# UCSC-nanopore-cgl/margin

Hardware: AMD Instinct MI355X
Metric: het-sites x reads phased/sec (30x ONT synthetic chunks, end to end: every merge level + final sweep) (higher is better)
Workload: dtype int32

## Files before the change

margin_amd/csrc/mrp_batch.cpp:

```cpp
#include <hip/hip_runtime.h>

#include <algorithm>
#include <array>
#include <cstdio>
#include <cstdlib>
#include <cstring>
#include <ctime>
#include <mutex>
#include <new>
#include <vector>

#include "mrp_internal.h"
#include "mrp_level_order.h"

extern "C" {

int mrp_batch_create(mrp_context *ctx, mrp_batch **out) {
    if (!ctx || !out) return mrp_set_error(MRP_ERR_ARG, "mrp_batch_create: bad arguments");
    mrp_batch *b = new (std::nothrow) mrp_batch();
    if (!b) return mrp_set_error(MRP_ERR_NOMEM, "out of host memory");
    b->ctx = ctx;
    b->bind_pool(&ctx->pool);
    *out = b;
    return MRP_OK;
// ... 332 lines not shown
    for (size_t i = 0; i < b->pcols.size(); i++) (b->pcols[i].need_planes ? plane_list : pack_list).push_back((int32_t) i);
    HIP_TRY(b->d_pack_list.upload(pack_list, s));
    HIP_TRY(b->d_plane_list.upload(plane_list, s));
    const double u3 = now_();
    const size_t nC = (size_t) b->n_cells_total;
    HIP_TRY(b->d_planes.alloc((size_t) b->n_slots * 8));
    HIP_TRY(b->d_slot_total.alloc((size_t) b->n_slots));
    HIP_TRY(b->d_slot_bytes.alloc((size_t) b->n_slots * 16));
    HIP_TRY(b->d_cost.alloc(nC));
    HIP_TRY(b->d_f32.alloc(nC));
    HIP_TRY(b->d_b32.alloc(nC));
    HIP_TRY(b->d_mf32.alloc((size_t) b->n_merge));
    HIP_TRY(b->d_mb32.alloc((size_t) b->n_merge));
    if (!b->order_f64.empty()) {
        HIP_TRY(b->d_f.alloc(nC));
        HIP_TRY(b->d_b.alloc(nC));
        HIP_TRY(b->d_mf.alloc((size_t) b->n_merge));
        HIP_TRY(b->d_mb.alloc((size_t) b->n_merge));
    }
    HIP_TRY(b->d_total.alloc(b->cols.size()));
    HIP_TRY(b->d_hmm_fb.alloc(2 * b->hmms.size()));
    const double u4 = now_();
    HIP_TRY(hipStreamSynchronize(s));
    if (timing_)
        fprintf(stderr, "      upload: plan %.2f ms, arrays %.2f, tiles+lists %.2f, allocs %.2f, sync %.2f\n", u1 - u0, u2 - u1, u3 - u2, u4 - u3, now_() - u4);

    b->dev = b->view();
    HostVec<int64_t>().swap(b->read_byte_off);
    HostVec<uint64_t>().swap(b->partition);
    HostVec<uint32_t>().swap(b->cell_next);
    HostVec<uint32_t>().swap(b->cell_prev);
    HostVec<uint32_t>().swap(b->cell_np);
    b->uploaded = true;
    return MRP_OK;
}

int mrp_batch_launch(mrp_batch *b) {
    if (!b) return mrp_set_error(MRP_ERR_ARG, "batch is NULL");
    if (!b->uploaded) {
        int rc = mrp_batch_upload(b);
        if (rc != MRP_OK) return rc;
    }
    mrp_context *ctx = b->ctx;
    HIP_TRY(hipSetDevice(ctx->device));
    hipStream_t s = ctx->stream;
    const MrpBatchDev &d = b->dev;
    hipStream_t ps = s;
    const size_t slot = (size_t) (b->n_launches % mrp_batch::EV_RING);
    if (slot >= b->ev_ring.size()) {
        std::array<hipEvent_t, 5> fresh{};
        for (auto &ev : fresh) HIP_TRY(hipEventCreate(&ev));
        b->ev_ring.push_back(fresh);
    }
    const std::array<hipEvent_t, 5> &ev = b->ev_ring[slot];
    if (b->n_launches >= mrp_batch::EV_RING) HIP_TRY(hipEventSynchronize(ev[2]));
    if (ps != s && ctx->last_emission) HIP_TRY(hipStreamWaitEvent(ps, ctx->last_emission, 0));
    HIP_TRY(hipEventRecord(ev[0], ps));
    HIP_TRY(mrp_launch_planes(d, ps));
    if (b->resident && mrp_dup('p')) HIP_TRY(mrp_launch_planes(d, ps));
    HIP_TRY(hipEventRecord(ev[1], ps));
    if (ps != s) HIP_TRY(hipStreamWaitEvent(s, ev[1], 0));
    HIP_TRY(hipEventRecord(ev[4], s));
    if (b->pre_sweep) HIP_TRY(b->pre_sweep(s));
    if (b->pre_sweep && mrp_dup('x')) HIP_TRY(b->pre_sweep(s));
    HIP_TRY(mrp_launch_emission(d, b->d_tiles.p, b->n_fast_tiles, b->n_tiles_dev - b->n_fast_tiles, s));
    HIP_TRY(hipEventRecord(ev[3], s));
    ctx->last_emission = ev[3];
    if (!b->order_f64.empty()) {
        const double neg = -__builtin_inf();
        HIP_TRY(mrp_launch_fill_f64(b->d_mf.p, d.n_merge, neg, s));
        HIP_TRY(mrp_launch_fill_f64(b->d_mb.p, d.n_merge, neg, s));
        HIP_TRY(mrp_launch_fill_f64(b->d_total.p, d.n_cols, neg, s));
        HIP_TRY(mrp_launch_fill_f64(b->d_hmm_fb.p, 2 * d.n_hmms, neg, s));
    }
    hipStream_t a0 = s, a1 = s;
    if (s == ctx->stream) HIP_TRY(ctx->side_streams(&a0, &a1));
    const bool side = a0 != s;
    if (side) {
        HIP_TRY(hipEventRecord(ctx->fork, s));
        HIP_TRY(hipStreamWaitEvent(a0, ctx->fork, 0));
        HIP_TRY(hipStreamWaitEvent(a1, ctx->fork, 0));
    }
    const int64_t chains = 2 * (int64_t) (b->order_wide.size() + b->order_mid.size()) * (int64_t) ctx->concurrent_batches;
    const int t_chain = ctx->concurrent_batches > 1 && chains > 2 * 256 ? 256 : 512;
    const int t_wide = t_chain, t_mid = t_chain, t_narrow = 64;
    HIP_TRY(mrp_launch_sweep_i32(d, b->d_order_wide.p, (int64_t) b->order_wide.size(), t_wide, b->max_merge_wide, s));
    HIP_TRY(mrp_launch_sweep_i32(d, b->d_order_mid.p, (int64_t) b->order_mid.size(), t_mid, b->max_merge_mid, a0));
    HIP_TRY(mrp_launch_sweep_i32(d, b->d_order_narrow.p, (int64_t) b->order_narrow.size(), t_narrow, b->max_merge_narrow, a1));
    if (b->resident && mrp_dup('s')) {
        HIP_TRY(mrp_launch_sweep_i32(d, b->d_order_wide.p, (int64_t) b->order_wide.size(), t_wide, b->max_merge_wide, s));
        HIP_TRY(mrp_launch_sweep_i32(d, b->d_order_mid.p, (int64_t) b->order_mid.size(), t_mid, b->max_merge_mid, a0));
        HIP_TRY(mrp_launch_sweep_i32(d, b->d_order_narrow.p, (int64_t) b->order_narrow.size(), t_narrow, b->max_merge_narrow, a1));
    }
    HIP_TRY(mrp_launch_sweep_f64(d, b->d_order_f64.p, (int64_t) b->order_gen.size(), 256, s));
    HIP_TRY(mrp_launch_sweep_lse(d, b->d_order_lse.p, (int64_t) b->order_lse.size(), b->max_merge_lse, s));
    HIP_TRY(mrp_launch_sweep_lse(d, b->d_order_lse_big.p, (int64_t) b->order_lse_big.size(), std::max(b->max_merge_lse_big, MRP_LSE_CUR_LDS_MAX_MERGE + 2), s));
    if (side) {
        HIP_TRY(hipEventRecord(ctx->join[0], a0));
        HIP_TRY(hipEventRecord(ctx->join[1], a1));
        HIP_TRY(hipStreamWaitEvent(s, ctx->join[0], 0));
        HIP_TRY(hipStreamWaitEvent(s, ctx->join[1], 0));
    }
    HIP_TRY(hipEventRecord(ev[2], s));
    b->n_launches++;
    b->launched = true;
    return MRP_OK;
}

int mrp_batch_stats(mrp_batch *b, mrp_launch_stats *out) {
    if (!b || !out) return mrp_set_error(MRP_ERR_ARG, "mrp_batch_stats: NULL argument");
    *out = b->stats;
    out->n_hmms_lse = (int64_t) (b->order_lse.size() + b->order_lse_big.size());
    out->n_hmms_generic = (int64_t) b->order_gen.size();
    out->n_hmms_int32 = (int64_t) (b->order_wide.size() + b->order_mid.size() + b->order_narrow.size());
    if (b->launched) {
        mrp_context *ctx = b->ctx;
        HIP_TRY(hipSetDevice(ctx->device));
        const int64_t k = std::min<int64_t>(std::max<int64_t>(b->n_launches - b->stats_mark, 1), std::min<int64_t>(b->n_launches, mrp_batch::EV_RING));
        b->stats_mark = b->n_launches;
        double sa = 0, se = 0, sc = 0;
        float a = 0, e = 0, c = 0;
        for (int64_t j = 0; j < k; j++) {
            const auto &ev = b->ev_ring[(size_t) ((b->n_launches - k + j) % mrp_batch::EV_RING)];
            HIP_TRY(hipEventSynchronize(ev[2]));
            HIP_TRY(hipEventElapsedTime(&a, ev[0], ev[1]));
            HIP_TRY(hipEventElapsedTime(&e, ev[4], ev[3]));
            HIP_TRY(hipEventElapsedTime(&c, ev[3], ev[2]));
            sa += a; se += e; sc += c;
        }
        out->planes_ms = a;
        out->emission_ms = e;
        out->sweep_ms = c;
        out->avg_planes_ms = k ? sa / (double) k : 0.0;
        out->avg_emission_ms = k ? se / (double) k : 0.0;
        out->avg_sweep_ms = k ? sc / (double) k : 0.0;
        out->launches_averaged = k;
    }
    return MRP_OK;
}

void mrp_batch_last_launch_ms(mrp_batch *b, float *pack, float *emission, float *recursion) {
    *pack = *emission = *recursion = 0.f;
    if (!b || !b->launched || b->n_launches < 1) return;
    const auto &ev = b->ev_ring[(size_t) ((b->n_launches - 1) % mrp_batch::EV_RING)];
    (void) hipEventElapsedTime(pack, ev[0], ev[1]);
    (void) hipEventElapsedTime(emission, ev[4], ev[3]);
    (void) hipEventElapsedTime(recursion, ev[3], ev[2]);
}

int mrp_batch_download(mrp_batch *b) {
    if (!b) return mrp_set_error(MRP_ERR_ARG, "batch is NULL");
    if (!b->launched) return mrp_set_error(MRP_ERR_ARG, "mrp_batch_download before mrp_batch_launch");
    mrp_context *ctx = b->ctx;
    HIP_TRY(hipSetDevice(ctx->device));
    hipStream_t s = ctx->stream;
    const MrpBatchDev &d = b->dev;
    const bool any_out = std::any_of(b->outs.begin(), b->outs.end(), [](const JobOut &o) { return o.cell_f != nullptr; });
    if (!any_out) {
        HIP_TRY(hipStreamSynchronize(s));
        return MRP_OK;
    }
    const bool has_f64 = !b->order_f64.empty();
    std::vector<double> f, bb, mf, mb, tot((size_t) d.n_cols), fb((size_t) (2 * d.n_hmms));
    std::vector<int32_t> f32((size_t) d.n_cells), b32((size_t) d.n_cells), mf32((size_t) d.n_merge), mb32((size_t) d.n_merge);
    if (has_f64) { f.resize((size_t) d.n_cells); bb.resize((size_t) d.n_cells); mf.resize((size_t) d.n_merge); mb.resize((size_t) d.n_merge); }
    auto pull = [&](void *h, const void *p, size_t bytes) -> hipError_t {
        if (bytes == 0) return hipSuccess;
// ... 159 lines not shown
```

margin_amd/csrc/mrp_context.cpp:

```cpp
#include <hip/hip_runtime.h>

#include <atomic>
#include <cstdarg>
#include <cstdio>
#include <cstdlib>
#include <mutex>
#include <new>

#include "mrp_internal.h"

static thread_local char g_err[512] = "";

extern "C" {

int mrp_set_error(int code, const char *fmt, ...) {
    va_list ap;
    va_start(ap, fmt);
    vsnprintf(g_err, sizeof(g_err), fmt, ap);
    va_end(ap);
    return code;
}

const char *mrp_last_error(void) { return g_err; }
const char *mrp_version(void) { return "margin_rphmm 0.5.0 gfx950"; }
// ... 41 lines not shown
    *device_held = ctx->pool.device >= 0 ? (int64_t) DevPoolRegistry::get().held[ctx->pool.device].load() : 0;
}
mrp_context *mrp_context_sibling(mrp_context *ctx, int i) {
    std::lock_guard<std::mutex> lock(ctx->sibling_mu);
    while ((int) ctx->siblings.size() <= i) {
        mrp_context *s = nullptr;
        if (mrp_context_create(ctx->device, &s) != MRP_OK) return nullptr;
        s->phase_groups = 1;
        s->grouped = true;
        s->test_hooks = ctx->test_hooks;
        ctx->siblings.push_back(s);
    }
    return ctx->siblings[(size_t) i];
}
int mrp_context_create(int device, mrp_context **out) {
    if (!out) return mrp_set_error(MRP_ERR_ARG, "mrp_context_create: out is NULL");
    *out = nullptr;
    int n = mrp_device_count();
    if (n <= 0) return mrp_set_error(MRP_ERR_NO_DEVICE, "no HIP device visible: the stRPHmm sweep has no CPU fallback");
    if (device < 0 || device >= n) return mrp_set_error(MRP_ERR_ARG, "device %d out of range (0..%d)", device, n - 1);
    HIP_TRY(hipSetDevice(device));
    mrp_context *ctx = new (std::nothrow) mrp_context();
    if (!ctx) return mrp_set_error(MRP_ERR_NOMEM, "out of host memory");
    ctx->device = device;
    ctx->pool.attach(device);
    hipError_t e = hipStreamCreateWithFlags(&ctx->stream, hipStreamNonBlocking);
    for (int i = 0; i < 4 && e == hipSuccess; i++) e = hipEventCreate(&ctx->ev[i]);
    if (e == hipSuccess) e = hipEventCreateWithFlags(&ctx->fork, hipEventDisableTiming);
    for (int i = 0; i < 2 && e == hipSuccess; i++) e = hipEventCreateWithFlags(&ctx->join[i], hipEventDisableTiming);
    if (e != hipSuccess) {
        mrp_context_destroy(ctx);
        return mrp_set_error(MRP_ERR_HIP, "context setup failed: %s", hipGetErrorString(e));
    }
    *out = ctx;
    return MRP_OK;
}

void mrp_context_destroy(mrp_context *ctx) {
    if (!ctx) return;
    for (mrp_context *s : ctx->siblings) mrp_context_destroy(s);
    ctx->siblings.clear();
    (void) hipSetDevice(ctx->device);
    mrp_engine_release_context_cache(ctx);
    (void) hipDeviceSynchronize();
    ctx->pool.destroy();
    for (auto &e : ctx->ev)
        if (e) (void) hipEventDestroy(e);
    if (ctx->fork) (void) hipEventDestroy(ctx->fork);
    if (ctx->block_ev) (void) hipEventDestroy(ctx->block_ev);
    for (auto &e : ctx->join)
        if (e) (void) hipEventDestroy(e);
    for (auto &st : ctx->aux)
        if (st) (void) hipStreamDestroy(st);
    if (ctx->pre) (void) hipStreamDestroy(ctx->pre);
    if (ctx->stream) (void) hipStreamDestroy(ctx->stream);
    delete ctx;
}

int mrp_context_trim(mrp_context *ctx) {
    if (!ctx) return mrp_set_error(MRP_ERR_ARG, "context is NULL");
    HIP_TRY(hipSetDevice(ctx->device));
    HIP_TRY(hipDeviceSynchronize());
    std::lock_guard<std::mutex> lock(ctx->sibling_mu);
    for (mrp_context *s_ : ctx->siblings) { s_->pool.reclaim(); s_->pool.trim(); }
    ctx->pool.reclaim();
    ctx->pool.trim();
    DevPoolRegistry::get().forget_budget(ctx->pool.device);
    return MRP_OK;
}

int mrp_context_synchronize(mrp_context *ctx) {
    if (!ctx) return mrp_set_error(MRP_ERR_ARG, "context is NULL");
    HIP_TRY(hipSetDevice(ctx->device));
    HIP_TRY(hipStreamSynchronize(ctx->stream));
    return MRP_OK;
}
int mrp_context_set_phase_groups(mrp_context *ctx, int groups) {
    if (!ctx || groups < 0 || groups > 16) return mrp_set_error(MRP_ERR_ARG, "mrp_context_set_phase_groups: bad arguments");
    ctx->phase_groups = groups;
    return MRP_OK;
}
int mrp_context_phase_groups(const mrp_context *ctx) { return ctx->phase_groups; }
int mrp_context_set_test_hooks(mrp_context *ctx, int hooks) {
    if (!ctx || hooks < 0 || hooks > 63) return mrp_set_error(MRP_ERR_ARG, "mrp_context_set_test_hooks: bad arguments");
    if ((hooks & 4) && ctx->pool.device >= 0) DevPoolRegistry::get().inject_oom[ctx->pool.device].store(1);
    hooks &= ~4;
    ctx->test_hooks = hooks;
    for (mrp_context *s_ : ctx->siblings) s_->test_hooks = hooks;
    return MRP_OK;
}
int mrp_context_test_hooks(const mrp_context *ctx) { return ctx->test_hooks; }

}
```

margin_amd/csrc/mrp_kernels.hip:

```cpp
#include <hip/hip_runtime.h>
#include <stdint.h>

#include "mrp_device.h"
#include "mrp_internal.h"
#include "mrp_kernels.h"
#include "../../include/margin_rphmm.h"

#define WAVE 64

#define K_AS(T) const __attribute__((address_space(4))) T *
#define K_PTR(T, p) ((K_AS(T)) (p))
template <typename T>
static __device__ __forceinline__ T k_load(const T *p) {
    static_assert(sizeof(T) % 4 == 0, "dword sized");
    T v;
    K_AS(uint32_t) s = K_PTR(uint32_t, p);
    uint32_t *dst = reinterpret_cast<uint32_t *>(&v);
#pragma unroll
    for (unsigned i = 0; i < sizeof(T) / 4; i++) dst[i] = s[i];
    return v;
}

static __device__ __forceinline__ double i32_to_log(int32_t v) {
    return v == MRP_NEG_I32 ? -__builtin_inf() : (double) v;
// ... 314 lines not shown
__global__ void __launch_bounds__(256) mrp_emission_kernel(MrpBatchDev d, const EmitTile *__restrict__ tiles,
                                                           int64_t n_tiles) {
    const int lane = threadIdx.x & (WAVE - 1);
    const int wave = __builtin_amdgcn_readfirstlane((int) (threadIdx.x / WAVE));
    const int64_t tile = (int64_t) blockIdx.x * (blockDim.x / WAVE) + wave;
    if (tile >= n_tiles) return;
    const EmitTile t = k_load(tiles + tile);
    if (t.depth <= 16) emit_tile<4, 4>(d, t, lane, 0);
    else if (t.depth <= 32) emit_tile<8, 4>(d, t, lane, 0);
    else if (t.depth <= 48) {
        emit_tile<12, 2>(d, t, lane, 0);
        if (t.n > 256) emit_tile<12, 2>(d, t, lane, 128);
    } else {
        emit_tile<16, 2>(d, t, lane, 0);
        if (t.n > 256) emit_tile<16, 2>(d, t, lane, 128);
    }
}

__global__ void __launch_bounds__(256) mrp_emission_general_kernel(MrpBatchDev d, const EmitTile *__restrict__ tiles,
                                                                   int64_t n_tiles) {
    const int lane = threadIdx.x & (WAVE - 1);
    const int wave = __builtin_amdgcn_readfirstlane((int) (threadIdx.x / WAVE));
    const int64_t tile = (int64_t) blockIdx.x * (blockDim.x / WAVE) + wave;
    if (tile >= n_tiles) return;
    const EmitTile t = k_load(tiles + tile);
    const DevCol c = k_load(d.cols + t.col);
    const DevChunk ch = k_load(d.chunks + c.chunk);
    K_AS(uint64_t) planes = K_PTR(uint64_t, d.planes);
    K_AS(uint32_t) slot_total = K_PTR(uint32_t, d.slot_total);
    const bool ancestor = (t.flags & MRP_FLAG_INCLUDE_ANCESTOR_SUB_PROB) != 0;
    for (int idx = lane; idx < t.n; idx += WAVE) {
        const uint64_t P[1] = {d.partition[t.cell_off + idx]};
        uint32_t cost[1];
        if (ancestor) cost[0] = column_cost_ancestor(c, ch, planes, slot_total, P[0]);
        else column_cost_plain<1, false>(c, K_PTR(uint32_t, ch.allele_number), planes, slot_total, P, cost);
        d.cell_cost[t.cell_off + idx] = cost[0];
    }
}

__global__ void __launch_bounds__(256) mrp_tiles_kernel(const DevCol *__restrict__ cols, const TileCol *__restrict__ tc, int64_t n_cols,
                                                        EmitTile *__restrict__ tiles) {
    const int64_t col = (int64_t) blockIdx.x * blockDim.x + threadIdx.x;
    if (col >= n_cols) return;
    const DevCol c = cols[col];
    const TileCol t0 = tc[col];
    int64_t at = t0.first;
    for (int32_t off = 0; off < c.n_cells; off += MRP_EMIT_TILE, at++) {
        EmitTile t;
        t.cell_off = c.cell_off + off;
        t.slot_off = c.slot_off;
        t.n = c.n_cells - off < MRP_EMIT_TILE ? c.n_cells - off : MRP_EMIT_TILE;
        t.col = (int32_t) col;
        t.n_sites = c.n_sites;
        t.uniform_alleles = t0.uniform_alleles;
        t.depth = c.depth;
        t.flags = c.flags;
        t.pad[0] = 0;
        t.pad[1] = 0;
        tiles[at] = t;
    }
}

hipError_t mrp_launch_tiles(const DevCol *cols_dev, const TileCol *tilecols_dev, int64_t n_cols, EmitTile *tiles_dev, hipStream_t stream) {
    if (n_cols <= 0) return hipSuccess;
    hipLaunchKernelGGL(mrp_tiles_kernel, dim3((unsigned) ((n_cols + 255) / 256)), dim3(256), 0, stream, cols_dev, tilecols_dev, n_cols, tiles_dev);
    return hipGetLastError();
}

hipError_t mrp_launch_emission(const MrpBatchDev &d, const EmitTile *tiles_dev, int64_t n_fast, int64_t n_general,
                               hipStream_t stream) {
    const int waves = 4;
    if (n_fast > 0)
        hipLaunchKernelGGL(mrp_emission_kernel, dim3((unsigned) ((n_fast + waves - 1) / waves)), dim3(waves * WAVE), 0,
                           stream, d, tiles_dev, n_fast);
    if (n_general > 0)
        hipLaunchKernelGGL(mrp_emission_general_kernel, dim3((unsigned) ((n_general + waves - 1) / waves)),
                           dim3(waves * WAVE), 0, stream, d, tiles_dev + n_fast, n_general);
    return hipGetLastError();
}

#define SWEEP_R 8
#define SWEEP_WIN 128

struct SweepShared {
    int32_t *cur;
    int32_t *nxt;
    int32_t *red;
    int2 *dsc;
    int win0;
};

static __device__ __forceinline__ void stage_window(SweepShared &S, const SweepCol *cols, int K, int win0, int tid, int T) {
    __syncthreads();
    for (int i = tid; i < SWEEP_WIN; i += T) {
        const int k = win0 + i;
        if (k >= 0 && k < K) S.dsc[i] = make_int2(cols[k].n_cells, cols[k].n_merge);
    }
    S.win0 = win0;
    __syncthreads();
}
static __device__ __forceinline__ int2 col_desc(const SweepShared &S, int k) {
    const int2 v = S.dsc[k - S.win0];
    return make_int2(__builtin_amdgcn_readfirstlane(v.x), __builtin_amdgcn_readfirstlane(v.y));
}

__global__ void __launch_bounds__(1024)
mrp_sweep_i32_kernel(MrpBatchDev d, const int32_t *__restrict__ order, int max_merge) {
    extern __shared__ __attribute__((aligned(16))) int32_t lds[];
    SweepShared S;
    S.cur = lds;
    S.nxt = lds + max_merge;
    S.red = lds + 2 * max_merge;
    S.dsc = reinterpret_cast<int2 *>(lds + 2 * max_merge + 4);
    S.win0 = 0;

    const int tid = threadIdx.x, T = blockDim.x, lane = threadIdx.x & (WAVE - 1);
    const bool backward = (blockIdx.x & 1) != 0;
    const int64_t hmm_index = K_PTR(int32_t, order)[blockIdx.x >> 1];
    const DevHmm h = k_load(d.hmms + hmm_index);
    const SweepCol *cols = d.scols + h.col0;
    const int K = h.n_cols;
    const SweepCol first_col = k_load(cols);
    const int N = (int) h.n_cells;
    const int G = (N + 3) / 4;
    const int Q = (G + T - 1) / T;
    const uint32_t *__restrict__ cost = d.cell_cost + first_col.cell_off;
    const uint32_t *__restrict__ np = d.cell_np + first_col.cell_off;
    int32_t *__restrict__ out_f = d.cell_f32 + first_col.cell_off;
    int32_t *__restrict__ out_b = d.cell_b32 + first_col.cell_off;
    int32_t *__restrict__ out_mf = d.merge_f32 + first_col.mcell_off;
    int32_t *__restrict__ out_mb = d.merge_b32 + first_col.mcell_off;

    typedef uint32_t u32x4 __attribute__((ext_vector_type(4)));
    typedef int32_t i32x4 __attribute__((ext_vector_type(4)));
    u32x4 rc0, rc1, rc2, rc3, rc4, rc5, rc6, rc7, rn0, rn1, rn2, rn3, rn4, rn5, rn6, rn7;
#define RING_LOAD(i, q)                                                                              \
    {                                                                                                \
        int g_ = (q) * T + tid;                                                                      \
        g_ = g_ < 0 ? 0 : (g_ > G - 1 ? G - 1 : g_);                                                 \
        asm volatile("global_load_dwordx4 %0, %2, off\n\tglobal_load_dwordx4 %1, %3, off"            \
                     : "=&v"(rc##i), "=&v"(rn##i)                                                    \
                     : "v"(cost + 4 * g_), "v"(np + 4 * g_)                                          \
                     : "memory");                                                                    \
    }
#ifdef MRP_SAFE_WAIT
#define RING_WAIT(i, n) asm volatile("s_waitcnt vmcnt(0)" : "+v"(rc##i), "+v"(rn##i)::"memory");
#else
#define RING_WAIT(i, n) asm volatile("s_waitcnt vmcnt(" #n ")" : "+v"(rc##i), "+v"(rn##i)::"memory");
#endif
    if (!backward) {
        RING_LOAD(0, 0) RING_LOAD(1, 1) RING_LOAD(2, 2) RING_LOAD(3, 3)
        RING_LOAD(4, 4) RING_LOAD(5, 5) RING_LOAD(6, 6) RING_LOAD(7, 7)
    } else {
        RING_LOAD(0, Q - 1) RING_LOAD(1, Q - 2) RING_LOAD(2, Q - 3) RING_LOAD(3, Q - 4)
        RING_LOAD(4, Q - 5) RING_LOAD(5, Q - 6) RING_LOAD(6, Q - 7) RING_LOAD(7, Q - 8)
    }

    for (int i = tid; i < 2 * max_merge; i += T) lds[i] = MRP_NEG_I32;
    if (tid < 4) S.red[tid] = MRP_NEG_I32;
    stage_window(S, cols, K, 0, tid, T);

#define STORE4(out, p0, ok, v)                                                                               \
    {                                                                                                        \
        int32_t *dst_ = (ok) ? (out) + (p0) : scratch;                                                       \
        const i32x4 q_ = {v[0], v[1], v[2], v[3]};                                                           \
        *reinterpret_cast<i32x4 *>(dst_) = q_;                                                               \
    }
    int32_t *scratch = d.cell_f32 + d.n_cells;

#define RING_DRAIN() asm volatile("s_waitcnt vmcnt(0)"                                                                          \
                 : "+v"(rc0), "+v"(rc1), "+v"(rc2), "+v"(rc3), "+v"(rc4), "+v"(rc5), "+v"(rc6), "+v"(rc7),       \
                   "+v"(rn0), "+v"(rn1), "+v"(rn2), "+v"(rn3), "+v"(rn4), "+v"(rn5), "+v"(rn6), "+v"(rn7)        \
                 :                                                                                             \
                 : "memory");

    if (!backward) {
        int k = 0;
        int2 dk = col_desc(S, 0);
        int cs = 0, ce = dk.x;
        int mo = 0;
        int32_t local_max = MRP_NEG_I32;
#define FWD_ROUND(i, qq, nw)                                                                               \
    RING_WAIT(i, nw)                                                                                         \
    {                                                                                                        \
    const int pos0 = 4 * ((qq) * T + tid);                                                                   \
    int32_t fv[4] = {MRP_NEG_I32, MRP_NEG_I32, MRP_NEG_I32, MRP_NEG_I32};                                    \
    if ((qq) < Q && k < K) {                                                                                 \
        const int rend = 4 * ((qq) + 1) * T;                                                                 \
        for (;;) {                                                                                           \
            const bool first = (k == 0), last = (k == K - 1);                                                \
                        \
            bool act[4];                                                                                     \
            bool any_act = false;                                                                            \
            _Pragma("unroll") for (int j = 0; j < 4; j++) {                                                  \
                const int p = pos0 + j;                                                                      \
                act[j] = (p >= cs) & (p < ce);                                                               \
                any_act |= act[j];                                                                           \
            }                                                                                                \
            if (__any(any_act)) {                                                                            \
                int32_t fp[4] = {0, 0, 0, 0};                                                                \
                if (!first) {                                                                                \
                    _Pragma("unroll") for (int j = 0; j < 4; j++)                                            \
                        fp[j] = S.cur[act[j] ? (rn##i[j] >> 16) : lane];           \
                }                                                                                            \
                _Pragma("unroll") for (int j = 0; j < 4; j++) {                                              \
                    const int32_t v = add_i32(fp[j], -(int32_t) rc##i[j]);                                   \
                    fv[j] = act[j] ? v : fv[j];                                                              \
                    const int32_t val = act[j] ? v : MRP_NEG_I32;                                            \
                    if (!last) atomicMax(&S.nxt[act[j] ? (rn##i[j] & 0xFFFFu) : lane], val);       \
                    else local_max = max(local_max, val);                                                    \
                }                                                                                            \
            }                                                                                                \
            if (ce > rend) break;                                \
                                                                                   \
            if (last) {                                                                                      \
                local_max = wave_max_i32(local_max);                                                         \
                if ((tid & (WAVE - 1)) == 0) atomicMax(&S.red[0], local_max);                                \
                k = K;                                                                                       \
                break;                                                                                       \
            }                                                                                                \
            if (k + 1 >= S.win0 + SWEEP_WIN) stage_window(S, cols, K, k, tid, T);                            \
            const int2 dn = col_desc(S, k + 1);                                                              \
            lds_barrier();                                                                                   \
            for (int m = tid; m < dk.y; m += T) out_mf[mo + m] = S.nxt[m];                       \
            if (k + 2 < K) for (int m = tid; m < dn.y; m += T) S.cur[m] = MRP_NEG_I32;                       \
            lds_barrier();                                                                                   \
            { int32_t *t_ = S.cur; S.cur = S.nxt; S.nxt = t_; }                                              \
            mo += dk.y;                                                                                      \
            k++;                                                                                             \
            dk = dn;                                                                                         \
            cs = ce;                                                                                         \
            ce = cs + dk.x;                                                                                  \
            if (cs >= rend) break;                                                                           \
        }                                                                                                    \
    }                                                                                                        \
    STORE4(out_f, pos0, (qq) < Q && pos0 < N, fv)                                                            \
    }                                                                                                        \
    RING_LOAD(i, (qq) + SWEEP_R)
        FWD_ROUND(0, 0, 14) FWD_ROUND(1, 1, 15) FWD_ROUND(2, 2, 16) FWD_ROUND(3, 3, 17)
        FWD_ROUND(4, 4, 18) FWD_ROUND(5, 5, 19) FWD_ROUND(6, 6, 20) FWD_ROUND(7, 7, 21)
        for (int q0 = SWEEP_R; q0 < Q; q0 += SWEEP_R) {
            FWD_ROUND(0, q0, 21) FWD_ROUND(1, q0 + 1, 21) FWD_ROUND(2, q0 + 2, 21) FWD_ROUND(3, q0 + 3, 21)
            FWD_ROUND(4, q0 + 4, 21) FWD_ROUND(5, q0 + 5, 21) FWD_ROUND(6, q0 + 6, 21) FWD_ROUND(7, q0 + 7, 21)
        }
#undef FWD_ROUND
        RING_DRAIN()
        __syncthreads();
        const double total = i32_to_log(S.red[0]);
        for (int kk = tid; kk < K; kk += T) d.col_total[h.col0 + kk] = total;
        if (tid == 0) d.hmm_fb[2 * hmm_index] = total;
    }
    else {
        int k = K - 1;
        if (k < S.win0 || k >= S.win0 + SWEEP_WIN) stage_window(S, cols, K, max(0, K - SWEEP_WIN), tid, T);
        int2 dk = col_desc(S, k);
        int ce = N, cs = N - dk.x;
        int mo = (int) h.n_merge;
        if (K >= 2) {
            if (k - 1 < S.win0) stage_window(S, cols, K, max(0, k - SWEEP_WIN + 1), tid, T);
            const int2 dp = col_desc(S, k - 1);
            for (int m = tid; m < dp.y; m += T) S.nxt[m] = MRP_NEG_I32;
        }
        lds_barrier();
        int32_t local_max = MRP_NEG_I32;
#define BWD_ROUND(i, qq, nw)                                                                                 \
    RING_WAIT(i, nw)                                                                                         \
    {                                                                                                        \
    const int pos0 = 4 * ((qq) * T + tid);                                                                   \
    int32_t bv[4] = {MRP_NEG_I32, MRP_NEG_I32, MRP_NEG_I32, MRP_NEG_I32};                                    \
    if ((qq) >= 0 && k >= 0) {                                                                               \
        const int rbeg = 4 * (qq) * T;                                                                       \
        for (;;) {                                                                                           \
            const bool first = (k == 0), last = (k == K - 1);                                                \
            bool act[4];                                                                                     \
            bool any_act = false;                                                                            \
            _Pragma("unroll") for (int j = 0; j < 4; j++) {                                                  \
                const int p = pos0 + j;                                                                      \
                act[j] = (p >= cs) & (p < ce);                                                               \
                any_act |= act[j];                                                                           \
            }                                                                                                \
            if (__any(any_act)) {                                                                            \
                int32_t bn[4] = {0, 0, 0, 0};                                                                \
                if (!last) {                                                                                 \
                    _Pragma("unroll") for (int j = 0; j < 4; j++)                                            \
                        bn[j] = S.cur[act[j] ? (rn##i[j] & 0xFFFFu) : lane];       \
                }                                                                                            \
                _Pragma("unroll") for (int j = 0; j < 4; j++) {                                              \
                    bv[j] = act[j] ? bn[j] : bv[j];                                                          \
                    const int32_t pv = act[j] ? add_i32(bn[j], -(int32_t) rc##i[j]) : MRP_NEG_I32;           \
                    if (!first) atomicMax(&S.nxt[act[j] ? (rn##i[j] >> 16) : lane], pv);                     \
                    else local_max = max(local_max, pv);                                                     \
                }                                                                                            \
            }                                                                                                \
            if (cs < rbeg) break;                            \
            if (first) {                                                                                     \
                local_max = wave_max_i32(local_max);                                                         \
                if ((tid & (WAVE - 1)) == 0) atomicMax(&S.red[1], local_max);                                \
                k = -1;                                                                                      \
                break;                                                                                       \
            }                                                                                                \
            if (k - 2 >= 0 && k - 2 < S.win0) stage_window(S, cols, K, max(0, k - SWEEP_WIN + 1), tid, T);   \
            else if (k - 1 < S.win0) stage_window(S, cols, K, max(0, k - SWEEP_WIN + 1), tid, T);            \
            const int2 dp = col_desc(S, k - 1);                                                              \
            const int n_clear = (k >= 2) ? col_desc(S, k - 2).y : 0;                                         \
            lds_barrier();                                                                                   \
            for (int m = tid; m < dp.y; m += T) out_mb[mo - dp.y + m] = S.nxt[m];                \
            for (int m = tid; m < n_clear; m += T) S.cur[m] = MRP_NEG_I32;                                   \
            lds_barrier();                                                                                   \
            { int32_t *t_ = S.cur; S.cur = S.nxt; S.nxt = t_; }                                              \
            mo -= dp.y;                                                                                      \
            k--;                                                                                             \
            dk = dp;                                                                                         \
            ce = cs;                                                                                         \
            cs = ce - dk.x;                                                                                  \
            if (ce <= rbeg) break;                                                                           \
        }                                                                                                    \
    }                                                                                                        \
    STORE4(out_b, pos0, (qq) >= 0 && pos0 < N, bv)                                                           \
    }                                                                                                        \
    RING_LOAD(i, (qq) - SWEEP_R)
        BWD_ROUND(0, Q - 1, 14) BWD_ROUND(1, Q - 2, 15) BWD_ROUND(2, Q - 3, 16) BWD_ROUND(3, Q - 4, 17)
        BWD_ROUND(4, Q - 5, 18) BWD_ROUND(5, Q - 6, 19) BWD_ROUND(6, Q - 7, 20) BWD_ROUND(7, Q - 8, 21)
        for (int q0 = Q - 1 - SWEEP_R; q0 >= 0; q0 -= SWEEP_R) {
            BWD_ROUND(0, q0, 21) BWD_ROUND(1, q0 - 1, 21) BWD_ROUND(2, q0 - 2, 21) BWD_ROUND(3, q0 - 3, 21)
            BWD_ROUND(4, q0 - 4, 21) BWD_ROUND(5, q0 - 5, 21) BWD_ROUND(6, q0 - 6, 21) BWD_ROUND(7, q0 - 7, 21)
        }
#undef BWD_ROUND
        RING_DRAIN()
        __syncthreads();
        if (tid == 0) d.hmm_fb[2 * hmm_index + 1] = i32_to_log(S.red[1]);
    }
#undef RING_DRAIN
#undef RING_LOAD
#undef RING_WAIT
#undef STORE4
}

hipError_t mrp_launch_sweep_i32(const MrpBatchDev &d, const int32_t *order_dev, int64_t n, int block_threads,
                                int max_merge, hipStream_t stream) {
    if (n == 0) return hipSuccess;
    if (max_merge < WAVE) max_merge = WAVE;
    const size_t lds = (size_t) (2 * max_merge + 4) * sizeof(int32_t) + SWEEP_WIN * sizeof(int2);
    auto k = mrp_sweep_i32_kernel;
    static PerDeviceOnce once;
    const hipError_t attr_status = once.run([] {
        return hipFuncSetAttribute((const void *) mrp_sweep_i32_kernel, hipFuncAttributeMaxDynamicSharedMemorySize, 160 * 1024);
    });
    if (attr_status != hipSuccess) return attr_status;
    hipLaunchKernelGGL(k, dim3((unsigned) (2 * n)), dim3(block_threads), lds, stream, d, order_dev, max_merge);
    return hipGetLastError();
}

static __device__ __forceinline__ double log_add_exact(double x, double y) {
    if (x == -__builtin_inf()) return y;
    if (y == -__builtin_inf()) return x;
    return x > y ? x + log(1.0 + exp(y - x)) : y + log(1.0 + exp(x - y));
}
static __device__ __forceinline__ double log_add_p(double a, double b, bool max_not_sum) {
    return max_not_sum ? (a > b ? a : b) : log_add_exact(a, b);
}
static __device__ __forceinline__ double load_agent(double *p) {
    return __hip_atomic_load(p, __ATOMIC_RELAXED, __HIP_MEMORY_SCOPE_AGENT);
}
static __device__ void atomic_log_add_p(double *addr, double v, bool max_not_sum) {
    if (v == -__builtin_inf()) return;
    unsigned long long *a = (unsigned long long *) addr;
    unsigned long long old = __hip_atomic_load(a, __ATOMIC_RELAXED, __HIP_MEMORY_SCOPE_AGENT);
    while (true) {
        const double cur = __longlong_as_double((long long) old);
        const double nv = log_add_p(cur, v, max_not_sum);
        const unsigned long long nvb = (unsigned long long) __double_as_longlong(nv);
        if (nvb == old) return;
        const unsigned long long seen = atomicCAS(a, old, nvb);
        if (seen == old) return;
        old = seen;
    }
}
static __device__ __forceinline__ double wave_log_add_p(double v, bool max_not_sum) {
#pragma unroll
    for (int o = 32; o > 0; o >>= 1) {
        const double t = __shfl_xor(v, o, WAVE);
        v = log_add_p(v, t, max_not_sum);
    }
    return v;
}

__global__ void __launch_bounds__(1024) mrp_sweep_f64_kernel(MrpBatchDev d, const int32_t *__restrict__ order) {
    const int tid = threadIdx.x, T = blockDim.x;
    const int64_t hmm_index = K_PTR(int32_t, order)[blockIdx.x];
    const DevHmm h = k_load(d.hmms + hmm_index);
    const SweepCol *cols = d.scols + h.col0;
    const int K = h.n_cols;
    const bool wide = h.wide_idx != 0;
    const bool max_not_sum = (h.flags & MRP_FLAG_MAX_NOT_SUM) != 0;
    const double NEG = -__builtin_inf();
    double *hmm_f = d.hmm_fb + 2 * hmm_index, *hmm_b = hmm_f + 1;

    for (int k = 0; k < K; k++) {
        const SweepCol c = k_load(cols + k);
        const bool first = (k == 0), last = (k == K - 1);
        const SweepCol pc = k_load(cols + (first ? k : k - 1));
        double local = NEG;
        for (int idx = tid; idx < c.n_cells; idx += T) {
            const int64_t g = c.cell_off + idx;
            const double e = -((double) d.cell_cost[g]);
            const uint32_t nx = wide ? d.cell_next[g] : (d.cell_np[g] & 0xFFFFu);
            const uint32_t pv = wide ? d.cell_prev[g] : (d.cell_np[g] >> 16);
            double fv = first ? 0.0 : load_agent(&d.merge_f[pc.mcell_off + pv]);
            fv += e;
            d.cell_f[g] = fv;
            if (!last) atomic_log_add_p(&d.merge_f[c.mcell_off + nx], fv, max_not_sum);
            else local = log_add_p(local, fv, max_not_sum);
        }
        if (last) {
            local = wave_log_add_p(local, max_not_sum);
            if ((tid & (WAVE - 1)) == 0) atomic_log_add_p(hmm_f, local, max_not_sum);
        }
        __syncthreads();
    }
    for (int k = K - 1; k >= 0; k--) {
        const SweepCol c = k_load(cols + k);
        const bool first = (k == 0), last = (k == K - 1);
        const SweepCol pc = k_load(cols + (first ? k : k - 1));
        double local_b = NEG, local_t = NEG;
        for (int idx = tid; idx < c.n_cells; idx += T) {
            const int64_t g = c.cell_off + idx;
            const uint32_t nx = wide ? d.cell_next[g] : (d.cell_np[g] & 0xFFFFu);
            const uint32_t pv = wide ? d.cell_prev[g] : (d.cell_np[g] >> 16);
            double p = -((double) d.cell_cost[g]);
            double bv = 0.0;
            if (!last) { bv = load_agent(&d.merge_b[c.mcell_off + nx]); p += bv; }
            d.cell_b[g] = bv;
            if (!first) atomic_log_add_p(&d.merge_b[pc.mcell_off + pv], p, max_not_sum);
// ... 198 lines not shown
```

Before: 416.5 million.

## Template i32 sweep kernel on block size and direction, keep column descriptors in registers

The i32 forward/backward sweep kernel is templated on block size and direction, with separate launch instantiations for 64, 256 and 512 threads. Column descriptors now sit in a per-wave register window filled by inline-asm global loads and read via readlane, with a three-column lookahead. This replaces the LDS staging window and the block-wide barriers it needed, and the per-cell work is split into edge and non-edge template variants so interior columns skip the first/last checks. It also adds a test hook that forces 256-thread chains, and it raises register pressure and adds a synchronous load wait inside the loop.

Result: faster. 437.5 million, median of 5 (+5.0%).

```diff
diff --git a/margin_amd/csrc/mrp_batch.cpp b/margin_amd/csrc/mrp_batch.cpp
--- a/margin_amd/csrc/mrp_batch.cpp
+++ b/margin_amd/csrc/mrp_batch.cpp
@@ -438,7 +438,7 @@
         HIP_TRY(hipStreamWaitEvent(a1, ctx->fork, 0));
     }
     const int64_t chains = 2 * (int64_t) (b->order_wide.size() + b->order_mid.size()) * (int64_t) ctx->concurrent_batches;
-    const int t_chain = ctx->concurrent_batches > 1 && chains > 2 * 256 ? 256 : 512;
+    const int t_chain = (ctx->test_hooks & 64) || (ctx->concurrent_batches > 1 && chains > 2 * 256) ? 256 : 512;
     const int t_wide = t_chain, t_mid = t_chain, t_narrow = 64;
     HIP_TRY(mrp_launch_sweep_i32(d, b->d_order_wide.p, (int64_t) b->order_wide.size(), t_wide, b->max_merge_wide, s));
     HIP_TRY(mrp_launch_sweep_i32(d, b->d_order_mid.p, (int64_t) b->order_mid.size(), t_mid, b->max_merge_mid, a0));
diff --git a/margin_amd/csrc/mrp_context.cpp b/margin_amd/csrc/mrp_context.cpp
--- a/margin_amd/csrc/mrp_context.cpp
+++ b/margin_amd/csrc/mrp_context.cpp
@@ -147,7 +147,7 @@
 }
 int mrp_context_phase_groups(const mrp_context *ctx) { return ctx->phase_groups; }
 int mrp_context_set_test_hooks(mrp_context *ctx, int hooks) {
-    if (!ctx || hooks < 0 || hooks > 63) return mrp_set_error(MRP_ERR_ARG, "mrp_context_set_test_hooks: bad arguments");
+    if (!ctx || hooks < 0 || hooks > 127) return mrp_set_error(MRP_ERR_ARG, "mrp_context_set_test_hooks: bad arguments");
     if ((hooks & 4) && ctx->pool.device >= 0) DevPoolRegistry::get().inject_oom[ctx->pool.device].store(1);
     hooks &= ~4;
     ctx->test_hooks = hooks;
diff --git a/margin_amd/csrc/mrp_kernels.hip b/margin_amd/csrc/mrp_kernels.hip
--- a/margin_amd/csrc/mrp_kernels.hip
+++ b/margin_amd/csrc/mrp_kernels.hip
@@ -420,40 +420,84 @@
 #define SWEEP_R 8
 #define SWEEP_WIN 128
 
-struct SweepShared {
-    int32_t *cur;
-    int32_t *nxt;
-    int32_t *red;
-    int2 *dsc;
-    int win0;
-};
-
-static __device__ __forceinline__ void stage_window(SweepShared &S, const SweepCol *cols, int K, int win0, int tid, int T) {
-    __syncthreads();
-    for (int i = tid; i < SWEEP_WIN; i += T) {
-        const int k = win0 + i;
-        if (k >= 0 && k < K) S.dsc[i] = make_int2(cols[k].n_cells, cols[k].n_merge);
-    }
-    S.win0 = win0;
-    __syncthreads();
-}
-static __device__ __forceinline__ int2 col_desc(const SweepShared &S, int k) {
-    const int2 v = S.dsc[k - S.win0];
-    return make_int2(__builtin_amdgcn_readfirstlane(v.x), __builtin_amdgcn_readfirstlane(v.y));
-}
-
-__global__ void __launch_bounds__(1024)
-mrp_sweep_i32_kernel(MrpBatchDev d, const int32_t *__restrict__ order, int max_merge) {
+typedef uint32_t u32x4 __attribute__((ext_vector_type(4)));
+typedef int32_t i32x4 __attribute__((ext_vector_type(4)));
+typedef uint32_t u32x2 __attribute__((ext_vector_type(2)));
+
+template <bool EDGE>
+static __device__ __forceinline__ void sweep_fwd_cells(const u32x4 rc, const u32x4 rn, int rel, int n, int lane, bool first, bool last,
+                                                       const int32_t *cur, int32_t *nxt, int32_t (&fv)[4], int32_t &local_max) {
+    bool act[4];
+    bool any_act = false;
+#pragma unroll
+    for (int j = 0; j < 4; j++) {
+        act[j] = (uint32_t) (rel + j) < (uint32_t) n;
+        any_act |= act[j];
+    }
+    if (!__any(any_act)) return;
+    int32_t fp[4] = {0, 0, 0, 0};
+    if (!EDGE || !first) {
+#pragma unroll
+        for (int j = 0; j < 4; j++) fp[j] = cur[act[j] ? (rn[j] >> 16) : (uint32_t) lane];
+    }
+#pragma unroll
+    for (int j = 0; j < 4; j++) {
+        const int32_t v = add_i32(fp[j], -(int32_t) rc[j]);
+        fv[j] = act[j] ? v : fv[j];
+        const int32_t val = act[j] ? v : MRP_NEG_I32;
+        if (!EDGE || !last) atomicMax(&nxt[act[j] ? (rn[j] & 0xFFFFu) : (uint32_t) lane], val);
+        else local_max = max(local_max, val);
+    }
+}
+template <bool EDGE>
+static __device__ __forceinline__ void sweep_bwd_cells(const u32x4 rc, const u32x4 rn, int rel, int n, int lane, bool first, bool last,
+                                                       const int32_t *cur, int32_t *nxt, int32_t (&bv)[4], int32_t &local_max) {
+    bool act[4];
+    bool any_act = false;
+#pragma unroll
+    for (int j = 0; j < 4; j++) {
+        act[j] = (uint32_t) (rel + j) < (uint32_t) n;
+        any_act |= act[j];
+    }
+    if (!__any(any_act)) return;
+    int32_t bn[4] = {0, 0, 0, 0};
+    if (!EDGE || !last) {
+#pragma unroll
+        for (int j = 0; j < 4; j++) bn[j] = cur[act[j] ? (rn[j] & 0xFFFFu) : (uint32_t) lane];
+    }
+#pragma unroll
+    for (int j = 0; j < 4; j++) {
+        bv[j] = act[j] ? bn[j] : bv[j];
+        const int32_t pv = act[j] ? add_i32(bn[j], -(int32_t) rc[j]) : MRP_NEG_I32;
+        if (!EDGE || !first) atomicMax(&nxt[act[j] ? (rn[j] >> 16) : (uint32_t) lane], pv);
+        else local_max = max(local_max, pv);
+    }
+}
+template <int T>
+static __device__ __forceinline__ void sweep_copy_out(int32_t *__restrict__ dst, const int32_t *src, int n, int lane, int wv0) {
+    for (int m0 = wv0; m0 < n; m0 += T) {
+        const int m = m0 + lane;
+        if (m < n) dst[m] = src[m];
+    }
+}
+template <int T>
+static __device__ __forceinline__ void sweep_wipe(int32_t *dst, int n, int lane, int wv0) {
+    for (int m0 = wv0; m0 < n; m0 += T) {
+        const int m = m0 + lane;
+        if (m < n) dst[m] = MRP_NEG_I32;
+    }
+}
+
+template <int T, bool BACKWARD>
+static __device__ __forceinline__ void sweep_i32_walk(const MrpBatchDev &d, const int32_t *__restrict__ order, int max_merge) {
     extern __shared__ __attribute__((aligned(16))) int32_t lds[];
-    SweepShared S;
-    S.cur = lds;
-    S.nxt = lds + max_merge;
-    S.red = lds + 2 * max_merge;
-    S.dsc = reinterpret_cast<int2 *>(lds + 2 * max_merge + 4);
-    S.win0 = 0;
-
-    const int tid = threadIdx.x, T = blockDim.x, lane = threadIdx.x & (WAVE - 1);
-    const bool backward = (blockIdx.x & 1) != 0;
+    int32_t *cur = lds;
+    int32_t *nxt = lds + max_merge;
+    int32_t *red = lds + 2 * max_merge;
+
+    const int tid = threadIdx.x, lane = threadIdx.x & (WAVE - 1);
+    const int wv0 = __builtin_amdgcn_readfirstlane((int) (threadIdx.x & ~(WAVE - 1)));
+    constexpr bool backward = BACKWARD;
     const int64_t hmm_index = K_PTR(int32_t, order)[blockIdx.x >> 1];
     const DevHmm h = k_load(d.hmms + hmm_index);
     const SweepCol *cols = d.scols + h.col0;
@@ -469,8 +513,31 @@
     int32_t *__restrict__ out_mf = d.merge_f32 + first_col.mcell_off;
     int32_t *__restrict__ out_mb = d.merge_b32 + first_col.mcell_off;
 
-    typedef uint32_t u32x4 __attribute__((ext_vector_type(4)));
-    typedef int32_t i32x4 __attribute__((ext_vector_type(4)));
+    u32x2 w0, w1;
+    int wb;
+#define WIN_FILL(base)                                                                               \
+    {                                                                                                \
+        wb = (base);                                                                                 \
+        int c0_ = wb + lane, c1_ = wb + WAVE + lane;                                                 \
+        c0_ = c0_ < 0 ? 0 : (c0_ > K - 1 ? K - 1 : c0_);                                             \
+        c1_ = c1_ < 0 ? 0 : (c1_ > K - 1 ? K - 1 : c1_);                                             \
+         \
+        asm volatile("global_load_dwordx2 %0, %2, off\n\tglobal_load_dwordx2 %1, %3, off\n\ts_waitcnt vmcnt(0)"  \
+                     : "=&v"(w0), "=&v"(w1)                                                          \
+                     : "v"(&cols[c0_].n_cells), "v"(&cols[c1_].n_cells)                              \
+                     : "memory");                                                                    \
+    }
+#define DESC_STEP_FWD(j) if ((j) >= wb + SWEEP_WIN) WIN_FILL(wb + SWEEP_WIN)
+#define DESC_STEP_BWD(j) if ((j) < wb) WIN_FILL(wb - SWEEP_WIN)
+#define DESC_GET(j, ox, oy)                                                                          \
+    {                                                                                                \
+        const int l_ = (j) - wb;                                                                     \
+        const int ax_ = __builtin_amdgcn_readlane((int) w0.x, l_ & (WAVE - 1)), ay_ = __builtin_amdgcn_readlane((int) w0.y, l_ & (WAVE - 1)); \
+        const int bx_ = __builtin_amdgcn_readlane((int) w1.x, l_ & (WAVE - 1)), by_ = __builtin_amdgcn_readlane((int) w1.y, l_ & (WAVE - 1)); \
+        ox = l_ < WAVE ? ax_ : bx_;                                                                  \
+        oy = l_ < WAVE ? ay_ : by_;                                                                  \
+    }
+
     u32x4 rc0, rc1, rc2, rc3, rc4, rc5, rc6, rc7, rn0, rn1, rn2, rn3, rn4, rn5, rn6, rn7;
 #define RING_LOAD(i, q)                                                                              \
     {                                                                                                \
@@ -495,8 +562,8 @@
     }
 
     for (int i = tid; i < 2 * max_merge; i += T) lds[i] = MRP_NEG_I32;
-    if (tid < 4) S.red[tid] = MRP_NEG_I32;
-    stage_window(S, cols, K, 0, tid, T);
+    if (tid < 4) red[tid] = MRP_NEG_I32;
+    lds_barrier();
 
 #define STORE4(out, p0, ok, v)                                                                               \
     {                                                                                                        \
@@ -512,11 +579,16 @@
                  :                                                                                             \
                  : "memory");
 
-    if (!backward) {
+    int dkx, dky, d1x, d1y, d2x, d2y;
+    if constexpr (!backward) {
         int k = 0;
-        int2 dk = col_desc(S, 0);
-        int cs = 0, ce = dk.x;
+        WIN_FILL(0)
+        DESC_GET(0, dkx, dky)
+        DESC_GET(1, d1x, d1y)
+        DESC_GET(2, d2x, d2y)
+        int cs = 0, ce = dkx;
         int mo = 0;
+        bool edge = true;
         int32_t local_max = MRP_NEG_I32;
 #define FWD_ROUND(i, qq, nw)                                                                               \
     RING_WAIT(i, nw)                                                                                         \
@@ -526,49 +598,30 @@
     if ((qq) < Q && k < K) {                                                                                 \
         const int rend = 4 * ((qq) + 1) * T;                                                                 \
         for (;;) {                                                                                           \
-            const bool first = (k == 0), last = (k == K - 1);                                                \
-                        \
-            bool act[4];                                                                                     \
-            bool any_act = false;                                                                            \
-            _Pragma("unroll") for (int j = 0; j < 4; j++) {                                                  \
-                const int p = pos0 + j;                                                                      \
-                act[j] = (p >= cs) & (p < ce);                                                               \
-                any_act |= act[j];                                                                           \
-            }                                                                                                \
-            if (__any(any_act)) {                                                                            \
-                int32_t fp[4] = {0, 0, 0, 0};                                                                \
-                if (!first) {                                                                                \
-                    _Pragma("unroll") for (int j = 0; j < 4; j++)                                            \
-                        fp[j] = S.cur[act[j] ? (rn##i[j] >> 16) : lane];           \
-                }                                                                                            \
-                _Pragma("unroll") for (int j = 0; j < 4; j++) {                                              \
-                    const int32_t v = add_i32(fp[j], -(int32_t) rc##i[j]);                                   \
-                    fv[j] = act[j] ? v : fv[j];                                                              \
-                    const int32_t val = act[j] ? v : MRP_NEG_I32;                                            \
-                    if (!last) atomicMax(&S.nxt[act[j] ? (rn##i[j] & 0xFFFFu) : lane], val);       \
-                    else local_max = max(local_max, val);                                                    \
-                }                                                                                            \
-            }                                                                                                \
+            if (edge) sweep_fwd_cells<true>(rc##i, rn##i, pos0 - cs, dkx, lane, k == 0, k == K - 1, cur, nxt, fv, local_max); \
+            else sweep_fwd_cells<false>(rc##i, rn##i, pos0 - cs, dkx, lane, false, false, cur, nxt, fv, local_max); \
             if (ce > rend) break;                                \
                                                                                    \
-            if (last) {                                                                                      \
+            if (k == K - 1) {                                                                                \
                 local_max = wave_max_i32(local_max);                                                         \
-                if ((tid & (WAVE - 1)) == 0) atomicMax(&S.red[0], local_max);                                \
+                if (lane == 0) atomicMax(&red[0], local_max);                                                \
                 k = K;                                                                                       \
                 break;                                                                                       \
             }                                                                                                \
-            if (k + 1 >= S.win0 + SWEEP_WIN) stage_window(S, cols, K, k, tid, T);                            \
-            const int2 dn = col_desc(S, k + 1);                                                              \
+            int d3x, d3y;                                                                                    \
+            DESC_STEP_FWD(k + 3)                                                                             \
+            DESC_GET(k + 3, d3x, d3y)                                                                        \
             lds_barrier();                                                                                   \
-            for (int m = tid; m < dk.y; m += T) out_mf[mo + m] = S.nxt[m];                       \
-            if (k + 2 < K) for (int m = tid; m < dn.y; m += T) S.cur[m] = MRP_NEG_I32;                       \
+            sweep_copy_out<T>(out_mf + mo, nxt, dky, lane, wv0);                                             \
+            if (k + 2 < K) sweep_wipe<T>(cur, d1y, lane, wv0);                                               \
             lds_barrier();                                                                                   \
-            { int32_t *t_ = S.cur; S.cur = S.nxt; S.nxt = t_; }                                              \
-            mo += dk.y;                                                                                      \
+            { int32_t *t_ = cur; cur = nxt; nxt = t_; }                                                      \
+            mo += dky;                                                                                       \
             k++;                                                                                             \
-            dk = dn;                                                                                         \
+            dkx = d1x; dky = d1y; d1x = d2x; d1y = d2y; d2x = d3x; d2y = d3y;                                \
             cs = ce;                                                                                         \
-            ce = cs + dk.x;                                                                                  \
+            ce = cs + dkx;                                                                                   \
+            edge = (k == K - 1);                                                                             \
             if (cs >= rend) break;                                                                           \
         }                                                                                                    \
     }                                                                                                        \
@@ -584,22 +637,21 @@
 #undef FWD_ROUND
         RING_DRAIN()
         __syncthreads();
-        const double total = i32_to_log(S.red[0]);
+        const double total = i32_to_log(red[0]);
         for (int kk = tid; kk < K; kk += T) d.col_total[h.col0 + kk] = total;
         if (tid == 0) d.hmm_fb[2 * hmm_index] = total;
     }
     else {
         int k = K - 1;
-        if (k < S.win0 || k >= S.win0 + SWEEP_WIN) stage_window(S, cols, K, max(0, K - SWEEP_WIN), tid, T);
-        int2 dk = col_desc(S, k);
-        int ce = N, cs = N - dk.x;
+        WIN_FILL((K - 1) & ~(SWEEP_WIN - 1))
+        DESC_GET(k, dkx, dky)
+        DESC_STEP_BWD(k - 1)
+        DESC_GET(k - 1, d1x, d1y)
+        DESC_STEP_BWD(k - 2)
+        DESC_GET(k - 2, d2x, d2y)
+        int ce = N, cs = N - dkx;
         int mo = (int) h.n_merge;
-        if (K >= 2) {
-            if (k - 1 < S.win0) stage_window(S, cols, K, max(0, k - SWEEP_WIN + 1), tid, T);
-            const int2 dp = col_desc(S, k - 1);
-            for (int m = tid; m < dp.y; m += T) S.nxt[m] = MRP_NEG_I32;
-        }
-        lds_barrier();
+        bool edge = true;
         int32_t local_max = MRP_NEG_I32;
 #define BWD_ROUND(i, qq, nw)                                                                                 \
     RING_WAIT(i, nw)                                                                                         \
@@ -609,48 +661,30 @@
     if ((qq) >= 0 && k >= 0) {                                                                               \
         const int rbeg = 4 * (qq) * T;                                                                       \
         for (;;) {                                                                                           \
-            const bool first = (k == 0), last = (k == K - 1);                                                \
-            bool act[4];                                                                                     \
-            bool any_act = false;                                                                            \
-            _Pragma("unroll") for (int j = 0; j < 4; j++) {                                                  \
-                const int p = pos0 + j;                                                                      \
-                act[j] = (p >= cs) & (p < ce);                                                               \
-                any_act |= act[j];                                                                           \
-            }                                                                                                \
-            if (__any(any_act)) {                                                                            \
-                int32_t bn[4] = {0, 0, 0, 0};                                                                \
-                if (!last) {                                                                                 \
-                    _Pragma("unroll") for (int j = 0; j < 4; j++)                                            \
-                        bn[j] = S.cur[act[j] ? (rn##i[j] & 0xFFFFu) : lane];       \
-                }                                                                                            \
-                _Pragma("unroll") for (int j = 0; j < 4; j++) {                                              \
-                    bv[j] = act[j] ? bn[j] : bv[j];                                                          \
-                    const int32_t pv = act[j] ? add_i32(bn[j], -(int32_t) rc##i[j]) : MRP_NEG_I32;           \
-                    if (!first) atomicMax(&S.nxt[act[j] ? (rn##i[j] >> 16) : lane], pv);                     \
-                    else local_max = max(local_max, pv);                                                     \
-                }                                                                                            \
-            }                                                                                                \
+            if (edge) sweep_bwd_cells<true>(rc##i, rn##i, pos0 - cs, dkx, lane, k == 0, k == K - 1, cur, nxt, bv, local_max); \
+            else sweep_bwd_cells<false>(rc##i, rn##i, pos0 - cs, dkx, lane, false, false, cur, nxt, bv, local_max); \
             if (cs < rbeg) break;                            \
-            if (first) {                                                                                     \
+            if (k == 0) {                                                                                    \
                 local_max = wave_max_i32(local_max);                                                         \
-                if ((tid & (WAVE - 1)) == 0) atomicMax(&S.red[1], local_max);                                \
+                if (lane == 0) atomicMax(&red[1], local_max);                                                \
                 k = -1;                                                                                      \
                 break;                                                                                       \
             }                                                                                                \
-            if (k - 2 >= 0 && k - 2 < S.win0) stage_window(S, cols, K, max(0, k - SWEEP_WIN + 1), tid, T);   \
-            else if (k - 1 < S.win0) stage_window(S, cols, K, max(0, k - SWEEP_WIN + 1), tid, T);            \
-            const int2 dp = col_desc(S, k - 1);                                                              \
-            const int n_clear = (k >= 2) ? col_desc(S, k - 2).y : 0;                                         \
+            int d3x, d3y;                                                                                    \
+            DESC_STEP_BWD(k - 3)                                                                             \
+            DESC_GET(k - 3, d3x, d3y)                                                                        \
+            const int n_clear = (k >= 2) ? d2y : 0;                                                          \
             lds_barrier();                                                                                   \
-            for (int m = tid; m < dp.y; m += T) out_mb[mo - dp.y + m] = S.nxt[m];                \
-            for (int m = tid; m < n_clear; m += T) S.cur[m] = MRP_NEG_I32;                                   \
+            sweep_copy_out<T>(out_mb + (mo - d1y), nxt, d1y, lane, wv0);                                     \
+            sweep_wipe<T>(cur, n_clear, lane, wv0);                                                          \
             lds_barrier();                                                                                   \
-            { int32_t *t_ = S.cur; S.cur = S.nxt; S.nxt = t_; }                                              \
-            mo -= dp.y;                                                                                      \
+            { int32_t *t_ = cur; cur = nxt; nxt = t_; }                                                      \
+            mo -= d1y;                                                                                       \
             k--;                                                                                             \
-            dk = dp;                                                                                         \
+            dkx = d1x; dky = d1y; d1x = d2x; d1y = d2y; d2x = d3x; d2y = d3y;                                \
             ce = cs;                                                                                         \
-            cs = ce - dk.x;                                                                                  \
+            cs = ce - dkx;                                                                                   \
+            edge = (k == 0);                                                                                 \
             if (ce <= rbeg) break;                                                                           \
         }                                                                                                    \
     }                                                                                                        \
@@ -666,27 +700,48 @@
 #undef BWD_ROUND
         RING_DRAIN()
         __syncthreads();
-        if (tid == 0) d.hmm_fb[2 * hmm_index + 1] = i32_to_log(S.red[1]);
+        if (tid == 0) d.hmm_fb[2 * hmm_index + 1] = i32_to_log(red[1]);
     }
 #undef RING_DRAIN
 #undef RING_LOAD
 #undef RING_WAIT
 #undef STORE4
+#undef WIN_FILL
+#undef DESC_STEP_FWD
+#undef DESC_STEP_BWD
+#undef DESC_GET
+}
+
+template <int T>
+__global__ void __launch_bounds__(T, 4)
+mrp_sweep_i32_kernel(MrpBatchDev d, const int32_t *__restrict__ order, int max_merge) {
+    if (blockIdx.x & 1) sweep_i32_walk<T, true>(d, order, max_merge);
+    else sweep_i32_walk<T, false>(d, order, max_merge);
+}
+
+template <int T>
+static hipError_t sweep_i32_launch(const MrpBatchDev &d, const int32_t *order_dev, int64_t n, size_t lds, int max_merge, hipStream_t stream) {
+    static PerDeviceOnce once;
+    const hipError_t attr_status = once.run([] {
+        return hipFuncSetAttribute((const void *) mrp_sweep_i32_kernel<T>, hipFuncAttributeMaxDynamicSharedMemorySize, 160 * 1024);
+    });
+    if (attr_status != hipSuccess) return attr_status;
+    hipLaunchKernelGGL(mrp_sweep_i32_kernel<T>, dim3((unsigned) (2 * n)), dim3(T), lds, stream, d, order_dev, max_merge);
+    return hipGetLastError();
 }
 
 hipError_t mrp_launch_sweep_i32(const MrpBatchDev &d, const int32_t *order_dev, int64_t n, int block_threads,
                                 int max_merge, hipStream_t stream) {
+    if (block_threads != 64 && block_threads != 256 && block_threads != 512) return hipErrorInvalidValue;
     if (n == 0) return hipSuccess;
     if (max_merge < WAVE) max_merge = WAVE;
-    const size_t lds = (size_t) (2 * max_merge + 4) * sizeof(int32_t) + SWEEP_WIN * sizeof(int2);
-    auto k = mrp_sweep_i32_kernel;
-    static PerDeviceOnce once;
-    const hipError_t attr_status = once.run([] {
-        return hipFuncSetAttribute((const void *) mrp_sweep_i32_kernel, hipFuncAttributeMaxDynamicSharedMemorySize, 160 * 1024);
-    });
-    if (attr_status != hipSuccess) return attr_status;
-    hipLaunchKernelGGL(k, dim3((unsigned) (2 * n)), dim3(block_threads), lds, stream, d, order_dev, max_merge);
-    return hipGetLastError();
+    const size_t lds = (size_t) (2 * max_merge + 4) * sizeof(int32_t);
+    if (lds > (size_t) 160 * 1024) return hipErrorInvalidValue;
+    switch (block_threads) {
+    case 64: return sweep_i32_launch<64>(d, order_dev, n, lds, max_merge, stream);
+    case 256: return sweep_i32_launch<256>(d, order_dev, n, lds, max_merge, stream);
+    default: return sweep_i32_launch<512>(d, order_dev, n, lds, max_merge, stream);
+    }
 }
 
 static __device__ __forceinline__ double log_add_exact(double x, double y) {
```
